# tomvanbraeckel/amv-codec-tools

Hardware: AMD Instinct MI355X
Metric: AMV frames/sec/GPU (160x120 decode, bit-exact) (higher is better)
Workload: dtype int32; 1 GPU; 160x120 AMV decode, 160000-frame synthetic stream per GPU, chunks resident in HBM; parallelism=frame-range x1, frames_per_gpu=160000, stream=seeded synthetic source (BASELINE.md section 4), every frame

## Files before the change

amv-codec-tools_amd/csrc/amv_decode_sync.hip:

```cpp
#include <atomic>

#include "amv_kernels.h"
#include "amv_segment.h"

namespace amv {

namespace {

constexpr uint32_t kRingWords = 16;
constexpr uint32_t kNever = 0xffffffffu;

__device__ __forceinline__ void wave_sync() {
    __builtin_amdgcn_fence(__ATOMIC_SEQ_CST, "wavefront");
    __builtin_amdgcn_wave_barrier();
}

template <int kWidth>
__device__ __forceinline__ uint32_t seg_excl_sum(uint32_t v, uint32_t sub, uint32_t& total) {
    uint32_t x = v;
#pragma unroll
    for (int d = 1; d < kWidth; d <<= 1) {
        const uint32_t y = __shfl_up(x, d, kWidth);
        if (sub >= (uint32_t)d) x += y;
    }
// ... 74 lines not shown
                    }
                }
                wv[q] = make_uint4(w[0], w[1], w[2], w[3]);
            }
#pragma unroll
            for (uint32_t q = 0; q < kBurst; ++q) {
            const uint32_t t0 = b0 + q * kTile;
            if (t0 >= end) break;
            const uint32_t p0 = t0 + lane * 16u;
            const uint32_t w[4] = {wv[q].x, wv[q].y, wv[q].z, wv[q].w};
            uint32_t ff = 0;
#pragma unroll
            for (uint32_t j = 0; j < 4u; ++j) {
                const uint32_t t = ((w[j] & 0x7f7f7f7fu) + 0x01010101u) & w[j] & 0x80808080u;
                ff |= ((((t >> 7) * 0x00204081u) >> 21) & 15u) << (4u * j);
            }
            uint32_t valid = 0xffffu;
            if (t0 == 0u || t0 + kTile > end) {
                const uint32_t lo = first > p0 ? min(first - p0, 16u) : 0u, hi = end > p0 ? min(end - p0, 16u) : 0u;
                valid = ((1u << hi) - 1u) & ~((1u << lo) - 1u);
                ff &= ~((1u << lo) - 1u);
            }
            uint32_t back = wave_shr1(ff);
            if (lane == 0) back = carry;
            const uint32_t before = ((ff << 1) | (back >> 15)) & 0xffffu;
            uint32_t keep;
            if (!__any((ff & before) != 0u || (lane == 0 && (carry >> 14) == 3u))) {
                keep = valid & ~before;
            } else {
                const uint32_t hist = back | (ff << 16);
                keep = 0;
                bool deep = false;
#pragma unroll
                for (uint32_t j = 0; j < 16u; ++j) {
                    const uint32_t run = (uint32_t)__builtin_clz(~(hist << (16u - j)) | 1u);
                    deep = deep || run >= 16u + j;
                    keep |= (!(run & 1u) ? 1u : 0u) << j;
                }
                keep &= valid;
                if (__any(deep)) { retry = true; break; }
            }
            carry = __builtin_amdgcn_readlane(ff, kWave - 1);
            const uint32_t cnt = (uint32_t)__builtin_popcount(keep);
            const uint32_t upto = wave_incl_sum(cnt);
            const uint32_t tile_total = __builtin_amdgcn_readlane(upto, kWave - 1);
            uint32_t d = total + upto - cnt;
#pragma unroll
            for (uint32_t j = 0; j < 4u; ++j) {
                const uint32_t k4 = (keep >> (4u * j)) & 15u;
                const uint32_t packed = __builtin_amdgcn_perm(0u, w[j], s_pack[k4]);
                const uint32_t sh = (d & 3u) * 8u, wd = d >> 2;
                atomicOr(&ring[wd & (kRing - 1u)], packed << sh);
                atomicOr(&ring[(wd + 1u) & (kRing - 1u)], (packed >> 1) >> (31u - sh));
                d += (uint32_t)__builtin_popcount(k4);
            }
            total += tile_total;
            wave_sync();
            const uint32_t whole = total >> 2;
            for (uint32_t x = flushed + lane; x < whole; x += kWave) {
                const uint32_t v = ring[x & (kRing - 1u)];
                ring[x & (kRing - 1u)] = 0u;
                out[x] = __builtin_amdgcn_perm(0u, v, 0x00010203u);
            }
            flushed = whole;
            wave_sync();
            }
        }
        if (!retry) {
            wave_sync();
            const uint32_t x = flushed + lane;
            if (x < ((total + 15u) & ~15u) >> 2) out[x] = __builtin_amdgcn_perm(0u, ring[x & (kRing - 1u)], 0x00010203u);
        }
    }
    if (lane == 0) {
        ws_bytes[frame] = retry ? kNever : total;
        if (retry) retry_list[atomicAdd(retry_count, 1u)] = frame;
    }
}

namespace {

struct Stream {
    const uint32_t* g;
    uint32_t nwords;
    uint32_t* ring;
    uint32_t hi;
    uint4 pf0, pf1;
};

constexpr int kStrideWrite = 8;

__device__ __forceinline__ uint4 stream_piece(const Stream& s, uint32_t x) {
    uint4 v = make_uint4(0, 0, 0, 0);
    if (x < s.nwords) v = *reinterpret_cast<const uint4*>(s.g + x);
    return v;
}

__device__ __forceinline__ void stream_request(Stream& s) {
    s.pf0 = stream_piece(s, s.hi);
    s.pf1 = stream_piece(s, s.hi + 4u);
}

struct SegGeom {
    uint32_t mcu_cols;
    uint32_t per_row;
    uint32_t count;
};

template <uint32_t kFlush>
__device__ __forceinline__ void stage_put(uint32_t* stage, uint32_t pos, uint32_t word) {
    stage[(pos & (2u * kFlush - 1u)) * kWave] = word;
}

template <uint32_t kFlush>
__device__ __forceinline__ void stage_flush(const uint32_t* stage, uint32_t* __restrict__ rec, uint32_t from, uint32_t rec_cap) {
    const uint32_t* p = stage + (from & (2u * kFlush - 1u)) * kWave;
    uint4 v[kFlush / 4u];
#pragma unroll
    for (uint32_t q = 0; q < kFlush / 4u; ++q)
        v[q] = make_uint4(p[(4u * q) * kWave], p[(4u * q + 1u) * kWave], p[(4u * q + 2u) * kWave], p[(4u * q + 3u) * kWave]);
    if (from + kFlush <= rec_cap) {
#pragma unroll
        for (uint32_t q = 0; q < kFlush / 4u; ++q) *reinterpret_cast<uint4*>(rec + from + 4u * q) = v[q];
    }
}

}

struct SyncOut {
    uint32_t* rec;
    const uint32_t* rec_line;
    uint32_t* seg_start;
    uint32_t* lane_tab;
    SegGeom sg;
    uint32_t lane_stride;
    uint32_t* rec_count;
    uint32_t* retry_list;
    uint32_t* retry_count;
    uint32_t ok_in_blocks;
};


namespace {

constexpr uint32_t kFastRegion = kFastWords * 4u;
constexpr uint32_t kFastTableBytes = 4u * kFastRegion;
constexpr uint32_t kServicePace = 4u;
template <int L> constexpr uint32_t skip_pace() { return L >= 16 ? 1u : kServicePace; }
constexpr uint32_t kSlot = kWave * 4u;
constexpr uint32_t kFastRingBytes = (kRingWords + 1u) * kSlot;
constexpr uint32_t kFastSumBytes = 4u * kSlot;
constexpr uint32_t fast_stage_bytes(uint32_t flush) { return 2u * flush * kSlot; }
constexpr uint32_t fast_per_wave(uint32_t flush) { return fast_stage_bytes(flush) + kFastSumBytes + kFastRingBytes; }
constexpr uint32_t fast_waves(uint32_t flush) {
    const uint32_t w = (160u * 1024u - kFastTableBytes) / fast_per_wave(flush);
    return w > 16u ? 16u : w;
}

struct FastState {
    uint32_t t;
    uint32_t k;
    uint32_t j;
    uint32_t togo6;
    uint32_t rp8;
    uint32_t dc;
};

typedef __attribute__((address_space(3))) uint32_t lds_u32;
__device__ __forceinline__ uint32_t lds_get(uint32_t a) { return *(const lds_u32*)(uintptr_t)a; }
__device__ __forceinline__ void lds_put(uint32_t a, uint32_t v) { *(lds_u32*)(uintptr_t)a = v; }
__device__ __forceinline__ uint32_t shl3_add(uint32_t x, uint32_t y) {
    uint32_t d;
    asm("v_lshl_add_u32 %0, %1, 3, %2" : "=v"(d) : "v"(x), "v"(y));
    return d;
}

__device__ __forceinline__ void fast_ring_put(const Stream& s, uint32_t x, const uint4& v) {
    uint32_t* d = s.ring + (x & (kRingWords - 1u)) * kWave;
    d[0] = v.x; d[kWave] = v.y; d[2 * kWave] = v.z; d[3 * kWave] = v.w;
    if ((x & (kRingWords - 1u)) == 0u) s.ring[kRingWords * kWave] = v.x;
}

__device__ __forceinline__ void fast_open(Stream& s) {
    const uint4 a = stream_piece(s, 0u), b = stream_piece(s, 4u), c = stream_piece(s, 8u), d = stream_piece(s, 12u);
    fast_ring_put(s, 0u, a);
    fast_ring_put(s, 4u, b);
    fast_ring_put(s, 8u, c);
    fast_ring_put(s, 12u, d);
    s.hi = kRingWords;
    stream_request(s);
}

template <uint32_t kPace>
__device__ __forceinline__ void fast_service_paced(Stream& s, uint32_t w, bool alive, bool& have, uint32_t stride_no) {
    if (alive && w + 9u > s.hi) {
        do {
            if (!have) stream_request(s);
            fast_ring_put(s, s.hi, s.pf0);
            fast_ring_put(s, s.hi + 4u, s.pf1);
            s.hi += 8u;
            have = false;
        } while (w + 9u > s.hi);
    }
    if ((stride_no & (kPace - 1u)) == 0u) {
        if (alive && !have) {
            stream_request(s);
            have = true;
        }
    }
}

__device__ __forceinline__ uint32_t fast_window(uint32_t ringb, uint32_t t) {
    const uint32_t ra = shl3_add(t & 0x1e0u, ringb);
    return __builtin_amdgcn_alignbit(lds_get(ra), lds_get(ra + kSlot), ~t);
}

__device__ __forceinline__ uint32_t fast_lookup(const FastState& s, uint32_t v) {
    const uint32_t toff = (((3u * kFastRegion) >> s.j) & kFastRegion) | (~s.dc & (2u * kFastRegion));
    const uint32_t e1 = lds_get(((v >> 21) & 0x7fcu) | toff);
    const uint32_t x2 = max(v >> 16, kFastLongFirst - 1u);
    const uint32_t e2 = lds_get((x2 << 2) + (toff + (kFastM2Word * 4u - 4u * (kFastLongFirst - 1u))));
    return e1 | e2;
}

template <uint32_t kFlush, bool kLimit>
__device__ __forceinline__ void fast_stride(uint32_t ringb, uint32_t stageb, uint32_t sumb, uint32_t lim1, FastState& s, uint32_t& seen,
                                            uint32_t& worst) {
#pragma unroll
    for (int it = 0; it < kStrideWrite; ++it) {
        const uint32_t ca = (((2u * kSlot) >> s.j) & (3u * kSlot)) | sumb;
        const uint32_t sum = lds_get(ca);
        const uint32_t v = fast_window(ringb, s.t);
        __builtin_amdgcn_sched_barrier(0);
        uint32_t run = (uint32_t)((int32_t)s.togo6 >> 31);
        if (kLimit) run &= (uint32_t)((int32_t)(s.t - lim1) >> 31);
        const uint32_t e = fast_lookup(s, v) & run;
        seen |= e;
        const uint32_t used = e >> 24;
        const int x = __builtin_amdgcn_sbfe((int)v, 0u - used, e);
        const uint32_t full = __builtin_amdgcn_ubfe(0xffffffffu, 0u, e);
        const uint32_t val = (uint32_t)x - (full ^ (uint32_t)(x >> 31));
        s.t += used;
        const uint32_t kn = s.k + ((e >> 16) & 255u);
        worst = min(worst, kn - 65u);
        uint32_t dcn = (uint32_t)__builtin_amdgcn_sbfe((int)kn, 6u, 1u);
        asm("" : "+v"(dcn));
        lds_put(ca, sum + (val & s.dc));
        const uint32_t rv = val + (sum & s.dc);
        lds_put((s.rp8 & ((2u * kFlush - 1u) << 8)) | stageb, (rv << 16) | (s.togo6 & 0xfc0u) | (kn - 1u));
        s.rp8 += e & kFastEmit;
        s.k = kn & ~dcn;
        s.togo6 += kn & 64u;
        s.j = min(s.j + dcn, 5u);
        s.dc = dcn;
    }
}

template <bool kLimit>
__device__ __forceinline__ uint32_t fast_replay(uint32_t ringb, uint32_t lim1, FastState& s) {
    for (int it = 0; it < kStrideWrite; ++it) {
        if (s.togo6 == 0u) break;
        if (kLimit && (int32_t)(s.t - lim1) >= 0) break;
        const uint32_t e = fast_lookup(s, fast_window(ringb, s.t));
        if (e & kFastInvalid) return 1u;
        const uint32_t kn = s.k + ((e >> 16) & 255u);
        s.t += e >> 24;
        if (kn - 65u < 15u) return 2u;
        const bool end = (kn & 64u) != 0u;
        s.rp8 += e & kFastEmit;
        s.k = end ? 0u : kn;
        s.togo6 += kn & 64u;
        s.j = end ? (s.j == 0u ? 5u : s.j - 1u) : s.j;
        s.dc = end ? ~0u : 0u;
    }
    return 0u;
}

__device__ __forceinline__ void fast_open_at(Stream& s, uint32_t w) {
    const uint32_t lo = w & ~7u;
    const uint4 a = stream_piece(s, lo), b = stream_piece(s, lo + 4u), c = stream_piece(s, lo + 8u), d = stream_piece(s, lo + 12u);
    fast_ring_put(s, lo, a);
    fast_ring_put(s, lo + 4u, b);
    fast_ring_put(s, lo + 8u, c);
    fast_ring_put(s, lo + 12u, d);
    s.hi = lo + kRingWords;
    stream_request(s);
}

template <uint32_t kPace>
__device__ __forceinline__ void fast_skip(Stream& win, uint32_t ringb, FastState& s, uint32_t lim1, uint32_t& nblk6, uint32_t& nrec8) {
    nblk6 = nrec8 = 0u;
    bool active = (int32_t)(s.t - lim1) < 0;
    if (!__ballot(active)) return;
    fast_open_at(win, active ? (s.t + 1u) >> 5 : 0u);
    bool have = true;
    uint32_t stride_no = 1u;
    while (__ballot(active) != 0ull) {
        fast_service_paced<kPace>(win, (s.t + 1u) >> 5, active, have, stride_no++);
#pragma unroll
        for (int it = 0; it < kStrideWrite; ++it) {
            const uint32_t v = fast_window(ringb, s.t);
            const uint32_t e = fast_lookup(s, v) & (uint32_t)((int32_t)(s.t - lim1) >> 31);
            s.t += e >> 24;
            const uint32_t kn = s.k + ((e >> 16) & 255u);
            uint32_t dcn = (uint32_t)__builtin_amdgcn_sbfe((int)kn, 6u, 1u);
            asm("" : "+v"(dcn));
            nrec8 += e & kFastEmit;
            nblk6 += kn & 64u;
            s.k = kn & ~dcn;
            s.j = min(s.j + dcn, 5u);
            s.dc = dcn;
        }
        active = (int32_t)(s.t - lim1) < 0;
    }
}

}

template <uint32_t kFlush>
__global__ __launch_bounds__(kWave * 16) void amv_huffman_fast_kernel(
    const uint32_t* __restrict__ ws, const uint32_t* __restrict__ ws_bytes, uint32_t n,
    const uint32_t* __restrict__ list, const uint32_t* __restrict__ list_count,
    uint32_t blocks_per_frame, const uint32_t* __restrict__ ws_line,
    const HuffDecodeImage* __restrict__ img, SyncOut out, int32_t* __restrict__ status,
    uint32_t* __restrict__ nmcu_ok, uint32_t* __restrict__ queue, unsigned long long* __restrict__ stats) {
    static_assert(kFlush == 8u, "amv_huffman_fast_kernel stages a stride's eight record slots");
    extern __shared__ __attribute__((aligned(16))) uint8_t s_mem[];
    const uint32_t wave = threadIdx.x >> 6, lane = threadIdx.x & 63u, nwaves = blockDim.x >> 6;
    {
        const uint4* src = reinterpret_cast<const uint4*>(&img->fast[0][0]);
        uint4* dst = reinterpret_cast<uint4*>(s_mem);
        for (uint32_t i = threadIdx.x; i < kFastTableBytes / 16u; i += blockDim.x) dst[i] = src[i];
    }
    __syncthreads();
    const bool lds_at_zero = (uint32_t)(uintptr_t)(__attribute__((address_space(3))) uint8_t*)s_mem == 0u;
    const uint32_t stageb = kFastTableBytes + wave * fast_stage_bytes(kFlush) + lane * 4u;
    const uint32_t sumb = kFastTableBytes + nwaves * fast_stage_bytes(kFlush) + wave * kFastSumBytes + lane * 4u;
    const uint32_t ringb = kFastTableBytes + nwaves * (fast_stage_bytes(kFlush) + kFastSumBytes) + wave * kFastRingBytes + lane * 4u;
    uint32_t* const stage = reinterpret_cast<uint32_t*>(s_mem + stageb);
    if (list) n = *list_count;
    const uint32_t ntasks = (n + kWave - 1) / kWave;
    const SegGeom sg = out.sg;
    for (;;) {
        uint32_t task = 0;
        if (lane == 0) task = atomicAdd(queue, 1u);
        task = __shfl(task, 0);
        if (task >= ntasks) return;
        const uint32_t idx = task * kWave + lane;
        const uint32_t frame = idx < n ? (list ? list[idx] : idx) : kNever;
        uint32_t total = frame != kNever ? ws_bytes[frame] : kNever;
        if (!lds_at_zero && total != kNever) {
            out.retry_list[atomicAdd(out.retry_count, 1u)] = frame;
            total = kNever;
        }
        if (frame != kNever && total == kNever) out.rec_count[frame] = kNever;
        if (!lds_at_zero) continue;
        const bool live = total != kNever;
        const uint32_t fsafe = live ? frame : 0u;
        const uint32_t line0 = out.rec_line[fsafe];
        uint32_t* const rec = out.rec + (uint64_t)line0 * 32u;
        const uint32_t line1 = out.rec_line[fsafe + 1u];
        const uint32_t cap_rec = line1 > line0 ? (line1 - line0) * 32u : 0u;
        uint2* const seg_out = reinterpret_cast<uint2*>(out.seg_start) + (uint64_t)fsafe * (sg.count + 1u);
        const uint32_t valid_bits = live ? total * 8u : 0u;
        Stream win{ws + (uint64_t)ws_line[fsafe] * 4u, live ? ((total + 15u) >> 4) * 4u : 0u, reinterpret_cast<uint32_t*>(s_mem + ringb), 0u,
                   make_uint4(0, 0, 0, 0), make_uint4(0, 0, 0, 0)};
        fast_open(win);
        for (uint32_t c = 0; c < 3u; ++c) lds_put(sumb + c * kSlot, 0u);

        FastState s{0xffffffffu, 0u, 5u, live ? 0u - (blocks_per_frame << 6) : 0u, 0u, ~0u};
        bool alive = live;
        uint32_t stop = 0;
        uint32_t stride_no = 0;
        bool have_words = true;
        uint32_t recpos = 0;
        uint32_t seg_next = 0, seg_col = 0, seg_blk = 0;
        uint32_t end_blocks = 0;
#pragma unroll
        for (uint32_t q = 0; q < 2u * kFlush; ++q) stage_put<kFlush>(stage, q, kDummyRecord);
        if (__ballot(alive) != 0ull) do {
            const bool line_live = alive;
            uint4 line[8];
#pragma unroll
            for (int quarter = 0; quarter < 4; ++quarter) {
                fast_service_paced<kServicePace>(win, (s.t + 1u) >> 5, alive, have_words, stride_no);
                const bool running = alive;
                s.rp8 = stride_no << 11;
                const FastState start = s;
                uint32_t worst = ~0u, seen = 0u;
                fast_stride<kFlush, false>(ringb, stageb, sumb, 0u, s, seen, worst);
                const bool trouble = alive && (worst < 15u || (seen & kFastInvalid) != 0u);
                if (__ballot(trouble) != 0ull) {
                    if (trouble) {
                        s = start;
                        stop = fast_replay<false>(ringb, 0u, s);
                        alive = false;
                        for (uint32_t q = s.rp8 >> 8; q < stride_no * 8u + 8u; ++q) stage_put<kFlush>(stage, q, kDummyRecord);
                    }
                }
                if (alive && s.togo6 == 0u) { stop = 3u; alive = false; }
                stage_put<kFlush>(stage, s.rp8 >> 8, kDummyRecord);
                {
                    uint32_t* p = stage + ((stride_no & 1u) * kFlush) * kWave;
                    line[2 * quarter] = make_uint4(p[0], p[kWave], p[2 * kWave], p[3 * kWave]);
                    line[2 * quarter + 1] = make_uint4(p[4 * kWave], p[5 * kWave], p[6 * kWave], p[7 * kWave]);
#pragma unroll
                    for (uint32_t q = 0; q < 8u; ++q) p[q * kWave] = kDummyRecord;
                }
                bool hit = false;
                uint32_t blocks = 0;
                if (running) {
                    blocks = blocks_per_frame + (uint32_t)((int32_t)s.togo6 >> 6);
                    hit = seg_next < sg.count && blocks + (s.k ? 1u : 0u) > seg_blk;
                    if (!alive) { end_blocks = blocks; s.togo6 = 0u; }
                }
                if (__ballot(hit) != 0ull) {
                    if (hit) {
                        seg_out[seg_next++] = make_uint2(start.rp8 >> 8, s.rp8 >> 8);
                        const bool last = seg_col + 1u == sg.per_row;
                        seg_blk += 6u * (last ? sg.mcu_cols - seg_col * kSegMcus : kSegMcus);
                        seg_col = last ? 0u : seg_col + 1u;
                    }
                }
                ++stride_no;
            }
            if (line_live) {
                const uint32_t at = (stride_no - 4u) * 8u;
                if (at + 32u <= cap_rec) {
                    uint4* d = reinterpret_cast<uint4*>(rec + at);
#pragma unroll
                    for (int q = 0; q < 8; ++q) d[q] = line[q];
                }
                recpos = at + 32u;
            }
        } while (__ballot(alive) != 0ull);
        if (live) {
            const uint32_t bits = s.t + 1u + (stop == 1u ? 17u : 0u);
            uint32_t st = stop == 1u ? kStFormat : (stop == 2u ? kStOverrun : 0u);
            if (bits > valid_bits) st |= kStTruncated;
            reinterpret_cast<uint4*>(out.lane_tab)[(uint64_t)frame * out.lane_stride] = make_uint4(0u, 0u, 0u, 0u);
            for (uint32_t m = seg_next; m <= sg.count; ++m) seg_out[m] = make_uint2(recpos, recpos);
            if (stats) atomicAdd(&stats[0], 1ull);
            if (recpos > cap_rec) {
                out.rec_count[frame] = kNever;
                out.retry_list[atomicAdd(out.retry_count, 1u)] = frame;
            } else {
                status[frame] = (int32_t)st;
                nmcu_ok[frame] = out.ok_in_blocks ? end_blocks : end_blocks / 6u;
                out.rec_count[frame] = recpos;
            }
        }
    }
}

template <int L>
__global__ __launch_bounds__(kWave * 16) void amv_huffman_sync2_kernel(
    const uint32_t* __restrict__ ws, const uint32_t* __restrict__ ws_bytes, uint32_t n,
    const uint32_t* __restrict__ list, const uint32_t* __restrict__ list_count,
    uint32_t blocks_per_frame, const uint32_t* __restrict__ ws_line,
    const HuffDecodeImage* __restrict__ img, SyncOut out, int32_t* __restrict__ status,
    uint32_t* __restrict__ nmcu_ok, uint32_t* __restrict__ queue, unsigned long long* __restrict__ stats) {
    constexpr int kFrames = kWave / L;
    constexpr uint32_t kFlush = 8u;
    constexpr uint32_t kNoLimit = 0x7ffffffeu;
    extern __shared__ __attribute__((aligned(16))) uint8_t s_mem[];
    const uint32_t wave = threadIdx.x >> 6, lane = threadIdx.x & 63u, nwaves = blockDim.x >> 6;
    const uint32_t slot = lane / L, sub = lane % L;
    if (list && *list_count == 0u) return;
    {
        const uint4* src = reinterpret_cast<const uint4*>(&img->fast[0][0]);
        uint4* dst = reinterpret_cast<uint4*>(s_mem);
        for (uint32_t i = threadIdx.x; i < kFastTableBytes / 16u; i += blockDim.x) dst[i] = src[i];
    }
    __syncthreads();
    const bool lds_at_zero = (uint32_t)(uintptr_t)(__attribute__((address_space(3))) uint8_t*)s_mem == 0u;
    const uint32_t stageb = kFastTableBytes + wave * fast_stage_bytes(kFlush) + lane * 4u;
    const uint32_t sumb = kFastTableBytes + nwaves * fast_stage_bytes(kFlush) + wave * kFastSumBytes + lane * 4u;
    const uint32_t ringb = kFastTableBytes + nwaves * (fast_stage_bytes(kFlush) + kFastSumBytes) + wave * kFastRingBytes + lane * 4u;
    uint32_t* const stage = reinterpret_cast<uint32_t*>(s_mem + stageb);
    if (list) n = *list_count;
    const uint32_t ntasks = (n + kFrames - 1) / kFrames;
    const SegGeom sg = out.sg;
    for (;;) {
        uint32_t task = 0;
        if (lane == 0) task = atomicAdd(queue, 1u);
        task = __shfl(task, 0);
        if (task >= ntasks) return;

        const bool timing = stats != nullptr && lane == 0;
        unsigned long long tc[6] = {0, 0, 0, 0, 0, 0};
        unsigned long long wall0 = 0;
        if (timing) { tc[0] = tc[1] = clock64(); wall0 = wall_clock64(); }

        const uint32_t idx = task * kFrames + slot;
        const uint32_t frame = idx < n ? (list ? list[idx] : idx) : kNever;
        uint32_t total = frame != kNever ? ws_bytes[frame] : kNever;
        if (!lds_at_zero && total != kNever) {
            if (sub == 0) out.retry_list[atomicAdd(out.retry_count, 1u)] = frame;
            total = kNever;
        }
        if (frame != kNever && total == kNever && sub == 0) out.rec_count[frame] = kNever;
        if (!lds_at_zero) continue;
        const bool live = total != kNever;
        const uint32_t fsafe = live ? frame : 0u;
        const uint32_t line0 = out.rec_line[fsafe];
        uint32_t* const rec = out.rec + (uint64_t)line0 * 32u;
        const uint32_t line1 = out.rec_line[fsafe + 1u];
        const uint32_t cap_rec = line1 > line0 ? (line1 - line0) * 32u : 0u;
        uint2* const seg_out = reinterpret_cast<uint2*>(out.seg_start) + (uint64_t)fsafe * (sg.count + 1u);
        const uint32_t valid_bits = live ? total * 8u : 0u;
        Stream win{ws + (uint64_t)ws_line[fsafe] * 4u, live ? ((total + 15u) >> 4) * 4u : 0u, reinterpret_cast<uint32_t*>(s_mem + ringb), 0u,
                   make_uint4(0, 0, 0, 0), make_uint4(0, 0, 0, 0)};

        uint32_t S = ((valid_bits + L - 1) / L + 31u) & ~31u;
        if (S < 64u) S = 64u;
        constexpr uint32_t kMemo = 5u, kPend = 4u;
        constexpr uint32_t kGuess = 5u << 11;
        const uint32_t stage0 = stageb - lane * 4u, sum0 = sumb - lane * 4u, col0 = slot * L;
        const uint64_t seg = L == 64 ? ~0ull : (((1ull << (L & 63)) - 1ull) << (slot * L));
        auto col_addr = [&](uint32_t col, uint32_t w) { return (w < 16u ? stage0 + w * kSlot : sum0 + (w - 16u) * kSlot) + col * 4u; };
        const bool walks = live && sub != L - 1;
        uint32_t my_blocks6 = 0u, my_recs8 = 0u, seeded = 0u, rounds = 0u;
        lds_put(col_addr(lane, 19u), 0u);
        {
            FastState st{sub * S - 1u, 0u, 5u, 0u, 0u, ~0u};
            const uint32_t lim1 = walks ? (sub + 1u) * S - 1u : 0u;
            if (!walks) st.t = lim1;
            uint32_t b6, r8;
            fast_skip<skip_pace<L>()>(win, ringb, st, lim1, b6, r8);
            if (walks) {
                lds_put(col_addr(lane, 0u), kGuess | (((st.t - lim1) | (st.k << 5) | (st.j << 11)) << 16));
                lds_put(col_addr(lane, 1u), b6);
                lds_put(col_addr(lane, 2u), r8);
                lds_put(col_addr(lane, 19u), 1u);
            }
        }
        if (timing) tc[2] = clock64();
        constexpr uint32_t kNone = 7u;
        uint32_t final_at = kNone, final_code = kGuess;
        bool settled = !live;
        for (int round = 0; round < L + 1; ++round) {
            wave_sync();
            const uint32_t held = lds_get(col_addr(lane, 19u));
            const uint32_t left_n = sub ? lds_get(col_addr(lane - 1u, 19u)) : 0u;
            uint32_t mine[kMemo], cand[kMemo];
#pragma unroll
            for (uint32_t q = 0; q < kMemo; ++q) {
                const uint32_t a = lds_get(col_addr(lane, 3u * q)), b = lds_get(col_addr(sub ? lane - 1u : lane, 3u * q));
                mine[q] = q < held ? a : kNever;
                cand[q] = q < left_n ? b >> 16 : kNever;
            }
            uint32_t link = (kNone << 15) | (kNone << 18) | (kNone << 21);
#pragma unroll
            for (uint32_t qp = 0; qp < kMemo; ++qp) {
                uint32_t to = kNone;
#pragma unroll
                for (uint32_t q = 0; q < kMemo; ++q) to = (mine[q] != kNever && (mine[q] & 0xffffu) == cand[qp]) ? q : to;
                if (sub == L - 1) to = cand[qp] != kNever ? 0u : kNone;
                link |= to << (3u * qp);
            }
            if (sub == 0) link = 0u;
            if (!live) link = 0u;
#pragma unroll
            for (int d = 1; d < L; d <<= 1) {
                const uint32_t before = __shfl_up(link, d, L);
                uint32_t both = 0u;
#pragma unroll
                for (uint32_t f = 0; f < 8u; ++f) both |= ((link >> (3u * ((before >> (3u * f)) & 7u))) & 7u) << (3u * f);
                if (sub >= (uint32_t)d) link = both;
            }
            final_at = link & 7u;
// ... 96 lines not shown
        uint32_t all_blocks, all_recs;
        const uint32_t blk0 = seg_excl_sum<L>(my_blocks6 >> 6, sub, all_blocks);
        const uint32_t rec0 = seg_excl_sum<L>(((my_recs8 >> 8) + kFlush - 1u) & ~(kFlush - 1u), sub, all_recs);

        for (uint32_t c = 0; c < 3u; ++c) lds_put(sumb + c * kSlot, 0u);
        FastState s = entry;
        s.togo6 = (blk0 - blocks_per_frame) << 6;
        s.rp8 = rec0 << 8;
        bool alive = live && blk0 < blocks_per_frame;
        if (!alive) s.togo6 = 0u;
        const uint32_t wlim1 = sub == L - 1 ? kNoLimit : (sub + 1u) * S - 1u;
        const uint32_t dc_first = blk0 + (s.k ? 1u : 0u);
        uint32_t stop = 0;
        uint32_t flushed = rec0;
        uint32_t end_blocks = 0;
        uint32_t seg_next, seg_col, seg_blk;
        {
            const uint32_t m_first = (dc_first + 5u) / 6u;
            uint32_t row = m_first / sg.mcu_cols;
            const uint32_t col = m_first - row * sg.mcu_cols;
            seg_col = (col + kSegMcus - 1u) / kSegMcus;
            if (seg_col >= sg.per_row) { ++row; seg_col = 0u; }
            seg_next = row * sg.per_row + seg_col;
            seg_blk = (row * sg.mcu_cols + seg_col * kSegMcus) * 6u;
        }
        if (__ballot(alive) != 0ull) {
        fast_open_at(win, alive ? (s.t + 1u) >> 5 : 0u);
        bool have_words = true;
        uint32_t stride_no = 1u;
        do {
            fast_service_paced<kServicePace>(win, (s.t + 1u) >> 5, alive, have_words, stride_no++);
            if ((s.rp8 >> 8) - flushed >= kFlush) {
                stage_flush<kFlush>(stage, rec, flushed, cap_rec);
                flushed += kFlush;
            }
            const bool running = alive;
            const FastState start = s;
            uint32_t worst = ~0u, seen = 0u;
            fast_stride<kFlush, true>(ringb, stageb, sumb, wlim1, s, seen, worst);
            const bool trouble = alive && (worst < 15u || (seen & kFastInvalid) != 0u);
            if (__ballot(trouble) != 0ull) {
                if (trouble) {
                    s = start;
                    stop = fast_replay<true>(ringb, wlim1, s);
                    alive = false;
                }
            }
            if (alive && s.togo6 == 0u) { stop = 3u; alive = false; }
            if (alive && (int32_t)(s.t - wlim1) >= 0) alive = false;
            bool hit = false;
            if (running) {
                const uint32_t blocks = blocks_per_frame + (uint32_t)((int32_t)s.togo6 >> 6);
                hit = seg_next < sg.count && blocks + (s.k ? 1u : 0u) > seg_blk;
                if (!alive) { end_blocks = blocks; s.togo6 = 0u; }
            }
            if (__ballot(hit) != 0ull) {
                if (hit) {
                    seg_out[seg_next++] = make_uint2(start.rp8 >> 8, s.rp8 >> 8);
                    const bool last = seg_col + 1u == sg.per_row;
                    seg_blk += 6u * (last ? sg.mcu_cols - seg_col * kSegMcus : kSegMcus);
                    seg_col = last ? 0u : seg_col + 1u;
                }
            }
        } while (__ballot(alive) != 0ull);
        }
        const uint32_t recpos = s.rp8 >> 8;
        {
            const uint32_t end = (recpos + kFlush - 1u) & ~(kFlush - 1u);
            for (uint32_t q = recpos; q < end; ++q) stage_put<kFlush>(stage, q, kDummyRecord);
            while (flushed < end) {
                stage_flush<kFlush>(stage, rec, flushed, cap_rec);
                flushed += kFlush;
            }
        }
        if (timing) tc[4] = clock64();
        const uint32_t err = stop == 1u ? kStFormat : (stop == 2u ? kStOverrun : 0u);
        const uint32_t stop_p = s.t + 1u + (stop == 1u ? 17u : 0u);
        const uint64_t stop_mask = __ballot(stop != 0u) & seg;
        uint32_t st = 0, good_blocks = blocks_per_frame, rec_total = 0, seg_seen = 0;
        int stop_lane = 0;
        if (stop_mask) {
            stop_lane = __builtin_ctzll(stop_mask);
            const uint32_t e = __shfl(err, stop_lane);
            const uint32_t eb = __shfl(end_blocks, stop_lane);
            const uint32_t sp = __shfl(stop_p, stop_lane);
            rec_total = __shfl(recpos, stop_lane);
            seg_seen = __shfl(seg_next, stop_lane);
            st = e;
            if (e) good_blocks = eb;
            if (sp > valid_bits) st |= kStTruncated;
        } else {
            st = kStFormat; good_blocks = 0;
        }

        uint32_t tot;
        const uint32_t by = seg_excl_sum<L>(lds_get(sumb), sub, tot);
        const uint32_t bu = seg_excl_sum<L>(lds_get(sumb + kSlot), sub, tot);
        const uint32_t bv = seg_excl_sum<L>(lds_get(sumb + 2u * kSlot), sub, tot);
        if (live) {
            const bool real = (int)lane <= stop_lane && blk0 < blocks_per_frame;
            reinterpret_cast<uint4*>(out.lane_tab)[(uint64_t)frame * out.lane_stride + sub] = make_uint4(real ? dc_first : kNever, by, bu, bv);
            for (uint32_t m = seg_seen + sub; m <= sg.count; m += L) seg_out[m] = make_uint2(rec_total, rec_total);
        }
        uint32_t wave_rounds = rounds;
        if (stats) {
#pragma unroll
            for (int off = 32; off; off >>= 1) wave_rounds = max(wave_rounds, (uint32_t)__shfl_xor((int)wave_rounds, off));
        }
        if (timing) {
            tc[5] = clock64();
            for (int q = 0; q < 5; ++q) atomicAdd(&stats[4 + q], tc[q + 1] - tc[q]);
            atomicAdd(&stats[9], 1ull);
            if (task < kTraceTasks) {
                unsigned long long* tr = stats + kTraceBase + (unsigned long long)task * 8ull;
                tr[0] = wall0;
                tr[1] = wall_clock64();
                for (int q = 0; q < 4; ++q) tr[2 + q] = tc[q + 2] - tc[q + 1];
                tr[6] = wave_rounds | (unsigned long long)S << 32;
                tr[7] = (unsigned long long)blockIdx.x << 32 | (unsigned long long)wave << 16 | (unsigned long long)L;
            }
        }
        if (live && sub == 0) {
            if (stats) {
                atomicAdd(&stats[0], 1ull);
                atomicAdd(&stats[1], (unsigned long long)rounds);
                atomicMax(&stats[2], (unsigned long long)rounds);
            }
            if (rec_total > cap_rec || unsettled) {
                out.rec_count[frame] = kNever;
                out.retry_list[atomicAdd(out.retry_count, 1u)] = frame;
            } else {
                status[frame] = (int32_t)st;
                nmcu_ok[frame] = out.ok_in_blocks ? good_blocks : good_blocks / 6u;
                out.rec_count[frame] = rec_total | ((uint32_t)(L - 1) << 24);
            }
        }
    }
}

namespace {

template <uint32_t kFlush>
void launch_fast(const uint32_t* ws, const uint32_t* ws_bytes, uint32_t n, const uint32_t* list,
                 const uint32_t* list_count, const FrameGeom& g, const uint32_t* ws_line,
                 const HuffDecodeImage* d_img, const SyncOut& out, int32_t* status, uint32_t* nmcu_ok,
                 uint32_t* queue, unsigned long long* stats, uint32_t cus, hipStream_t s) {
    constexpr uint32_t kMaxWaves = fast_waves(kFlush);
    static std::atomic<uint64_t> raised{0};
    int dev = 0;
    (void)hipGetDevice(&dev);
    const uint64_t bit = 1ull << (dev & 63);
    if (!(raised.load(std::memory_order_relaxed) & bit)) {
        (void)hipFuncSetAttribute(reinterpret_cast<const void*>(amv_huffman_fast_kernel<kFlush>),
                                  hipFuncAttributeMaxDynamicSharedMemorySize, (int)(kFastTableBytes + kMaxWaves * fast_per_wave(kFlush)));
        raised.fetch_or(bit, std::memory_order_relaxed);
    }
    const uint32_t tasks = (n + (uint32_t)kWave - 1u) / (uint32_t)kWave;
    uint32_t waves = (tasks + cus - 1u) / cus;
    if (waves < 4u) waves = 4u;
    if (waves > kMaxWaves) waves = kMaxWaves;
    const uint32_t grid = tasks < cus ? tasks : cus;
    hipLaunchKernelGGL((amv_huffman_fast_kernel<kFlush>), dim3(grid), dim3(kWave * waves), kFastTableBytes + waves * fast_per_wave(kFlush), s,
                       ws, ws_bytes, n, list, list_count, g.blocks, ws_line, d_img, out, status, nmcu_ok, queue, stats);
}

template <int L>
void launch_sync2(const uint32_t* ws, const uint32_t* ws_bytes, uint32_t n, const uint32_t* list,
                  const uint32_t* list_count, const FrameGeom& g, const uint32_t* ws_line,
                  const HuffDecodeImage* d_img, const SyncOut& out, int32_t* status, uint32_t* nmcu_ok,
                  uint32_t* queue, unsigned long long* stats, uint32_t cus, hipStream_t s) {
    constexpr uint32_t kMaxWaves = fast_waves(8u);
    static std::atomic<uint64_t> raised{0};
    int dev = 0;
    (void)hipGetDevice(&dev);
    const uint64_t bit = 1ull << (dev & 63);
    if (!(raised.load(std::memory_order_relaxed) & bit)) {
        (void)hipFuncSetAttribute(reinterpret_cast<const void*>(amv_huffman_sync2_kernel<L>),
                                  hipFuncAttributeMaxDynamicSharedMemorySize, (int)(kFastTableBytes + kMaxWaves * fast_per_wave(8u)));
        raised.fetch_or(bit, std::memory_order_relaxed);
    }
    const uint32_t tasks = (n + (uint32_t)(kWave / L) - 1u) / (uint32_t)(kWave / L);
    uint32_t waves = (tasks + cus - 1u) / cus;
    if (waves < 4u) waves = 4u;
    if (waves > kMaxWaves) waves = kMaxWaves;
    const uint32_t grid = tasks < cus ? tasks : cus;
    hipLaunchKernelGGL((amv_huffman_sync2_kernel<L>), dim3(grid), dim3(kWave * waves), kFastTableBytes + waves * fast_per_wave(8u), s, ws,
                       ws_bytes, n, list, list_count, g.blocks, ws_line, d_img, out, status, nmcu_ok, queue, stats);
}

}

int huffman_sync_lanes(uint32_t n, uint32_t cus, int wanted, uint64_t pixels) {
    if (wanted == 1 || wanted == 2 || wanted == 4 || wanted == 8 || wanted == 16 || wanted == 32 || wanted == 64) return wanted;
    if (n >= cus * 230u) return 1;
    if (n >= cus * 150u) return 2;
    const uint64_t resident = (uint64_t)cus * fast_waves(8u);
    if (pixels <= 30000u && (uint64_t)n * 8u > resident * 64u) return 2;
    int full = 8;
    while (full < 64 && (uint64_t)full * 25000u <= pixels) full *= 2;
    int fill = 8;
    if (n <= resident) fill = 64;
    else if (n <= 2u * resident) fill = 32;
    else if (n <= 4u * resident) fill = 16;
    int cap = 8;
    while (cap < 64 && (uint64_t)cap * 2u * 500u <= pixels) cap *= 2;
    if (n <= cus * 5u) cap = 64;
    if (fill > cap) fill = cap;
    return fill > full ? fill : full;
}

__global__ __launch_bounds__(256) void amv_split_kernel(const uint32_t* __restrict__ lens, uint32_t n, const uint32_t* __restrict__ ws_line,
                                                        uint32_t* __restrict__ heavy, uint32_t* __restrict__ light, uint32_t* __restrict__ count) {
    const uint32_t i = blockIdx.x * 256u + threadIdx.x, lane = threadIdx.x & 63u;
    const bool in = i < n;
    const uint64_t all = ws_line[n];
    const bool is_heavy = in && (((uint64_t)lens[in ? i : 0u] + 47u) >> 4) * n > 2u * all;
    const uint64_t hm = __ballot(is_heavy), lm = __ballot(in && !is_heavy);
    uint32_t hb = 0u, lb = 0u;
    if (lane == 0u) {
        if (hm) hb = atomicAdd(&count[0], (uint32_t)__builtin_popcountll(hm));
        if (lm) lb = atomicAdd(&count[1], (uint32_t)__builtin_popcountll(lm));
    }
    hb = (uint32_t)__shfl((int)hb, 0);
    lb = (uint32_t)__shfl((int)lb, 0);
    const uint64_t below = (1ull << lane) - 1ull;
    if (is_heavy) heavy[hb + (uint32_t)__builtin_popcountll(hm & below)] = i;
    else if (in) light[lb + (uint32_t)__builtin_popcountll(lm & below)] = i;
}

void launch_split_by_weight(const uint32_t* lens, uint32_t n, const uint32_t* ws_line, uint32_t* heavy, uint32_t* light, uint32_t* count,
                            hipStream_t s) {
    if (n == 0) return;
    hipLaunchKernelGGL(amv_split_kernel, dim3((n + 255u) / 256u), dim3(256), 0, s, lens, n, ws_line, heavy, light, count);
}

void launch_unstuff(const uint8_t* blob, uint64_t blob_bytes, const uint64_t* offs, const uint32_t* lens, uint32_t n,
                    const uint32_t* ws_line, uint32_t* ws, uint32_t* ws_bytes, uint32_t* retry_list, uint32_t* retry_count,
                    hipStream_t s) {
    if (n == 0) return;
    hipLaunchKernelGGL(amv_unstuff_kernel, dim3((n + 3u) / 4u), dim3(256), 0, s, blob, blob_bytes, offs, lens, n,
                       ws_line, ws, ws_bytes, retry_list, retry_count);
}

void launch_huffman_sync(const uint32_t* ws, const uint32_t* ws_bytes, uint32_t n, const uint32_t* list,
                         const uint32_t* list_count, const FrameGeom& g, const uint32_t* ws_line, int lanes_per_frame,
                         const HuffDecodeImage* d_img, const SyncSinks& sinks, int32_t* status, uint32_t* nmcu_ok,
                         uint32_t* queue, unsigned long long* stats, uint32_t cus, hipStream_t s) {
    if (n == 0) return;
    const uint32_t per_row = segs_per_row(g);
    SyncOut out{sinks.rec, sinks.rec_line, sinks.seg_start, sinks.lane_tab, SegGeom{g.mcu_cols, per_row, per_row * g.mcu_rows},
                sinks.lanes, sinks.rec_count, sinks.retry_list, sinks.retry_count, sinks.ok_in_blocks};
#define AMV_SYNC_ARGS ws, ws_bytes, n, list, list_count, g, ws_line, d_img, out, status, nmcu_ok, queue, stats, cus, s
    switch (lanes_per_frame) {
        case 64: launch_sync2<64>(AMV_SYNC_ARGS); break;
        case 32: launch_sync2<32>(AMV_SYNC_ARGS); break;
        case 8: launch_sync2<8>(AMV_SYNC_ARGS); break;
        case 4: launch_sync2<4>(AMV_SYNC_ARGS); break;
        case 2: launch_sync2<2>(AMV_SYNC_ARGS); break;
        case 1: launch_fast<8>(AMV_SYNC_ARGS); break;
        default: launch_sync2<16>(AMV_SYNC_ARGS); break;
    }
#undef AMV_SYNC_ARGS
}

namespace {
constexpr uint32_t kLayoutBlock = 256;

__device__ __forceinline__ uint32_t layout_lines(uint32_t len, const LayoutSpec& sp) {
    const uint64_t want = ((uint64_t)len * sp.per_byte_x2 >> 1) + sp.add;
    return (uint32_t)((min(want, (uint64_t)sp.hi) + ((1u << sp.unit_shift) - 1u)) >> sp.unit_shift);
}

struct Sum2 { uint64_t x, y; };
__device__ __forceinline__ Sum2 block_scan2(uint2 v, Sum2* s_wave, Sum2& tot) {
    const uint32_t lane = threadIdx.x & 63u, wave = threadIdx.x >> 6;
    Sum2 inc{v.x, v.y};
#pragma unroll
    for (int d = 1; d < 64; d <<= 1) {
        const uint64_t ax = (uint64_t)__shfl_up((unsigned long long)inc.x, d), ay = (uint64_t)__shfl_up((unsigned long long)inc.y, d);
        if (lane >= (uint32_t)d) { inc.x += ax; inc.y += ay; }
    }
    if (lane == 63u) s_wave[wave] = inc;
    __syncthreads();
    Sum2 base{0u, 0u};
    tot = Sum2{0u, 0u};
    for (uint32_t k = 0; k < kLayoutBlock / 64u; ++k) {
        const Sum2 w = s_wave[k];
        if (k < wave) { base.x += w.x; base.y += w.y; }
        tot.x += w.x; tot.y += w.y;
    }
    return Sum2{base.x + inc.x - v.x, base.y + inc.y - v.y};
}
__device__ __forceinline__ uint32_t sat32(uint64_t v) { return (uint32_t)min(v, (uint64_t)0xffffffffu); }
}

__global__ __launch_bounds__(kLayoutBlock) void amv_layout_sums_kernel(const uint32_t* __restrict__ lens, uint32_t n, LayoutSpec a, LayoutSpec b,
                                                                      uint2* __restrict__ sums) {
    __shared__ Sum2 s_wave[kLayoutBlock / 64u];
    const uint32_t i = blockIdx.x * kLayoutBlock + threadIdx.x;
    const uint32_t len = i < n ? lens[i] : 0u;
    Sum2 tot;
    (void)block_scan2(i < n ? make_uint2(layout_lines(len, a), b.line ? layout_lines(len, b) : 0u) : make_uint2(0u, 0u), s_wave, tot);
    if (threadIdx.x == 0u) sums[blockIdx.x] = make_uint2(sat32(tot.x), sat32(tot.y));
}

__global__ __launch_bounds__(1024) void amv_layout_scan_kernel(uint2* __restrict__ sums, uint32_t nb, uint32_t cap_a, uint32_t cap_b) {
    __shared__ uint64_t s_x[1024], s_y[1024];
    const uint32_t per = (nb + 1023u) / 1024u;
    const uint32_t lo = min(threadIdx.x * per, nb), up = min(lo + per, nb);
    uint64_t mx = 0, my = 0;
    for (uint32_t i = lo; i < up; ++i) { mx += sums[i].x; my += sums[i].y; }
    s_x[threadIdx.x] = mx; s_y[threadIdx.x] = my;
    __syncthreads();
    for (uint32_t d = 1; d < 1024u; d <<= 1) {
        const uint64_t lx = threadIdx.x >= d ? s_x[threadIdx.x - d] : 0u, ly = threadIdx.x >= d ? s_y[threadIdx.x - d] : 0u;
// ... 120 lines not shown
```

amv-codec-tools_amd/csrc/amv_tables.h:

```cpp
#pragma once
#include <stdint.h>

namespace amv {

static constexpr uint8_t kQuantLuma[64] = {
    8,  6,  6,  7,  6,  5,  8,  7,  7,  7,  9,  9,  8,  10, 12, 20, 13, 12, 11, 11, 12, 25,
    18, 19, 15, 20, 29, 26, 31, 30, 29, 26, 28, 28, 32, 36, 46, 39, 32, 34, 44, 39, 28, 28,
    40, 55, 41, 44, 48, 49, 52, 52, 52, 31, 39, 57, 61, 56, 50, 60, 46, 51, 52, 50};
static constexpr uint8_t kQuantChroma[64] = {
    9,  9,  9,  12, 11, 12, 24, 13, 13, 24, 50, 33, 28, 33, 50, 50, 50, 50, 50, 50, 50, 50,
    50, 50, 50, 50, 50, 50, 50, 50, 50, 50, 50, 50, 50, 50, 50, 50, 50, 50, 50, 50, 50, 50,
    50, 50, 50, 50, 50, 50, 50, 50, 50, 50, 50, 50, 50, 50, 50, 50, 50, 50, 50, 50};

static constexpr uint8_t kQ60Luma[64] = {
    13, 9,  10, 11, 10, 8,  13, 11, 10, 11, 14, 14, 13, 15, 19, 32, 21, 19, 18, 18, 19, 39,
    28, 30, 23, 32, 46, 41, 49, 48, 46, 41, 45, 44, 51, 58, 74, 62, 51, 54, 70, 55, 44, 45,
    64, 87, 65, 70, 76, 78, 82, 83, 82, 50, 62, 90, 97, 90, 80, 96, 74, 81, 82, 79};
static constexpr uint8_t kQ60Chroma[64] = {
    14, 14, 14, 19, 17, 19, 38, 21, 21, 38, 79, 53, 45, 53, 79, 79, 79, 79, 79, 79, 79, 79,
    79, 79, 79, 79, 79, 79, 79, 79, 79, 79, 79, 79, 79, 79, 79, 79, 79, 79, 79, 79, 79, 79,
    79, 79, 79, 79, 79, 79, 79, 79, 79, 79, 79, 79, 79, 79, 79, 79, 79, 79, 79, 79};

static constexpr uint8_t kScanOfNatural[64] = {
    0,  1,  5,  6,  14, 15, 27, 28, 2,  4,  7,  13, 16, 26, 29, 42, 3,  8,  12, 17, 25, 30,
    41, 43, 9,  11, 18, 24, 31, 40, 44, 53, 10, 19, 23, 32, 39, 45, 52, 54, 20, 22, 33, 38,
    46, 51, 55, 60, 21, 34, 37, 47, 50, 56, 59, 61, 35, 36, 48, 49, 57, 58, 62, 63};
static constexpr int kAmvlibQuirkNatural = 3 * 8 + 4;
static constexpr int kAmvlibQuirkScan = 37;

static constexpr uint8_t kHuffCount[4][16] = {
    {0, 1, 5, 1, 1, 1, 1, 1, 1, 0, 0, 0, 0, 0, 0, 0},
    {0, 3, 1, 1, 1, 1, 1, 1, 1, 1, 1, 0, 0, 0, 0, 0},
    {0, 2, 1, 3, 3, 2, 4, 3, 5, 5, 4, 4, 0, 0, 1, 0x7d},
    {0, 2, 1, 2, 4, 4, 3, 4, 7, 5, 4, 4, 0, 1, 2, 0x77}};
static constexpr uint8_t kHuffDcSymbols[12] = {0, 1, 2, 3, 4, 5, 6, 7, 8, 9, 10, 11};
static constexpr uint8_t kHuffAcLumaSymbols[162] = {
    0x01, 0x02, 0x03, 0x00, 0x04, 0x11, 0x05, 0x12, 0x21, 0x31, 0x41, 0x06, 0x13, 0x51, 0x61,
    0x07, 0x22, 0x71, 0x14, 0x32, 0x81, 0x91, 0xa1, 0x08, 0x23, 0x42, 0xb1, 0xc1, 0x15, 0x52,
    0xd1, 0xf0, 0x24, 0x33, 0x62, 0x72, 0x82, 0x09, 0x0a, 0x16, 0x17, 0x18, 0x19, 0x1a, 0x25,
    0x26, 0x27, 0x28, 0x29, 0x2a, 0x34, 0x35, 0x36, 0x37, 0x38, 0x39, 0x3a, 0x43, 0x44, 0x45,
    0x46, 0x47, 0x48, 0x49, 0x4a, 0x53, 0x54, 0x55, 0x56, 0x57, 0x58, 0x59, 0x5a, 0x63, 0x64,
    0x65, 0x66, 0x67, 0x68, 0x69, 0x6a, 0x73, 0x74, 0x75, 0x76, 0x77, 0x78, 0x79, 0x7a, 0x83,
    0x84, 0x85, 0x86, 0x87, 0x88, 0x89, 0x8a, 0x92, 0x93, 0x94, 0x95, 0x96, 0x97, 0x98, 0x99,
    0x9a, 0xa2, 0xa3, 0xa4, 0xa5, 0xa6, 0xa7, 0xa8, 0xa9, 0xaa, 0xb2, 0xb3, 0xb4, 0xb5, 0xb6,
    0xb7, 0xb8, 0xb9, 0xba, 0xc2, 0xc3, 0xc4, 0xc5, 0xc6, 0xc7, 0xc8, 0xc9, 0xca, 0xd2, 0xd3,
    0xd4, 0xd5, 0xd6, 0xd7, 0xd8, 0xd9, 0xda, 0xe1, 0xe2, 0xe3, 0xe4, 0xe5, 0xe6, 0xe7, 0xe8,
    0xe9, 0xea, 0xf1, 0xf2, 0xf3, 0xf4, 0xf5, 0xf6, 0xf7, 0xf8, 0xf9, 0xfa};
static constexpr uint8_t kHuffAcChromaSymbols[162] = {
    0x00, 0x01, 0x02, 0x03, 0x11, 0x04, 0x05, 0x21, 0x31, 0x06, 0x12, 0x41, 0x51, 0x07, 0x61,
    0x71, 0x13, 0x22, 0x32, 0x81, 0x08, 0x14, 0x42, 0x91, 0xa1, 0xb1, 0xc1, 0x09, 0x23, 0x33,
    0x52, 0xf0, 0x15, 0x62, 0x72, 0xd1, 0x0a, 0x16, 0x24, 0x34, 0xe1, 0x25, 0xf1, 0x17, 0x18,
    0x19, 0x1a, 0x26, 0x27, 0x28, 0x29, 0x2a, 0x35, 0x36, 0x37, 0x38, 0x39, 0x3a, 0x43, 0x44,
    0x45, 0x46, 0x47, 0x48, 0x49, 0x4a, 0x53, 0x54, 0x55, 0x56, 0x57, 0x58, 0x59, 0x5a, 0x63,
    0x64, 0x65, 0x66, 0x67, 0x68, 0x69, 0x6a, 0x73, 0x74, 0x75, 0x76, 0x77, 0x78, 0x79, 0x7a,
    0x82, 0x83, 0x84, 0x85, 0x86, 0x87, 0x88, 0x89, 0x8a, 0x92, 0x93, 0x94, 0x95, 0x96, 0x97,
    0x98, 0x99, 0x9a, 0xa2, 0xa3, 0xa4, 0xa5, 0xa6, 0xa7, 0xa8, 0xa9, 0xaa, 0xb2, 0xb3, 0xb4,
    0xb5, 0xb6, 0xb7, 0xb8, 0xb9, 0xba, 0xc2, 0xc3, 0xc4, 0xc5, 0xc6, 0xc7, 0xc8, 0xc9, 0xca,
    0xd2, 0xd3, 0xd4, 0xd5, 0xd6, 0xd7, 0xd8, 0xd9, 0xda, 0xe2, 0xe3, 0xe4, 0xe5, 0xe6, 0xe7,
    0xe8, 0xe9, 0xea, 0xf2, 0xf3, 0xf4, 0xf5, 0xf6, 0xf7, 0xf8, 0xf9, 0xfa};

static constexpr int8_t kImaIndexAdjust[16] = {-1, -1, -1, -1, 2, 4, 6, 8, -1, -1, -1, -1, 2, 4, 6, 8};
static constexpr int16_t kImaStep[89] = {
    7,     8,     9,     10,    11,    12,    13,    14,    16,    17,    19,    21,    23,
    25,    28,    31,    34,    37,    41,    45,    50,    55,    60,    66,    73,    80,
    88,    97,    107,   118,   130,   143,   157,   173,   190,   209,   230,   253,   279,
    307,   337,   371,   408,   449,   494,   544,   598,   658,   724,   796,   876,   963,
    1060,  1166,  1282,  1411,  1552,  1707,  1878,  2066,  2272,  2499,  2749,  3024,  3327,
    3660,  4026,  4428,  4871,  5358,  5894,  6484,  7132,  7845,  8630,  9493,  10442, 11487,
    12635, 13899, 15289, 16818, 18500, 20350, 22385, 24623, 27086, 29794, 32767};

static constexpr int16_t kSinQ14[65] = {
    0,     402,   804,   1205,  1606,  2006,  2404,  2801,  3196,  3590,  3981,  4370,  4756,
    5139,  5520,  5897,  6270,  6639,  7005,  7366,  7723,  8076,  8423,  8765,  9102,  9434,
    9760,  10080, 10394, 10702, 11003, 11297, 11585, 11866, 12140, 12406, 12665, 12916, 13160,
    13395, 13623, 13842, 14053, 14256, 14449, 14635, 14811, 14978, 15137, 15286, 15426, 15557,
    15679, 15791, 15893, 15986, 16069, 16143, 16207, 16261, 16305, 16340, 16364, 16379, 16384};


static constexpr int kLut1Bits = 9;
static constexpr int kLut2Bits = 7;
static constexpr int kLut2Pages = 16;
static constexpr uint32_t kFastWords = 2048;
static constexpr uint32_t kFastM2Word = 512;
static constexpr uint32_t kFastLongFirst = 0xfc00u;
static constexpr uint32_t kFastInvalid = 1u << 5, kFastEmit = 1u << 8, kFastEobAdvance = 192u;
struct HuffDecodeImage {
    uint16_t l1[4][1 << kLut1Bits];
    uint16_t l2[kLut2Pages][1 << kLut2Bits];
    uint32_t fast[4][kFastWords];
};

struct HuffEncodeImage {
    uint32_t code[4][256];
};

struct FrameGeom {
    uint32_t width, height;
    uint32_t stride;
    uint32_t mcu_cols;
    uint32_t mcu_rows;
    uint32_t mcus;
    uint32_t blocks;
    uint64_t frame_bytes;
};

inline FrameGeom make_geom(uint32_t w, uint32_t h) {
    FrameGeom g;
    g.width = w;
    g.height = h;
    g.stride = (w * 24 + 31) / 32 * 4;
    g.mcu_cols = (w + 15) / 16;
    g.mcu_rows = (h + 15) / 16;
    g.mcus = g.mcu_cols * g.mcu_rows;
    g.blocks = g.mcus * 6;
    g.frame_bytes = (uint64_t)g.stride * h;
    return g;
}

}
```

Measured before the change: 30.44 million frames/s.

## Keep stride records in registers instead of LDS staging buffer

The Huffman fast kernel now writes each stride's eight record words into per-lane registers instead of scattering them into a per-wave LDS staging area and reading them back. Table entries are rewritten while loading into LDS so that invalid codes and no-value symbols are encoded in the entry itself, which lets a single min-based check detect trouble. The aim is to cut LDS traffic, LDS footprint and the per-stride dummy refills. The cost is higher register pressure, and dummy padding now covers every slot in the stride rather than only the emitted ones.

```diff
diff --git a/amv-codec-tools_amd/csrc/amv_decode_sync.hip b/amv-codec-tools_amd/csrc/amv_decode_sync.hip
--- a/amv-codec-tools_amd/csrc/amv_decode_sync.hip
+++ b/amv-codec-tools_amd/csrc/amv_decode_sync.hip
@@ -250,6 +250,7 @@
 constexpr uint32_t kFastSumBytes = 4u * kSlot;
 constexpr uint32_t fast_stage_bytes(uint32_t flush) { return 2u * flush * kSlot; }
 constexpr uint32_t fast_per_wave(uint32_t flush) { return fast_stage_bytes(flush) + kFastSumBytes + kFastRingBytes; }
+constexpr uint32_t lane_per_wave() { return kFastSumBytes + kFastRingBytes; }
 constexpr uint32_t fast_waves(uint32_t flush) {
     const uint32_t w = (160u * 1024u - kFastTableBytes) / fast_per_wave(flush);
     return w > 16u ? 16u : w;
@@ -313,7 +314,8 @@
     return __builtin_amdgcn_alignbit(lds_get(ra), lds_get(ra + kSlot), ~t);
 }
 
-__device__ __forceinline__ uint32_t fast_lookup(const FastState& s, uint32_t v) {
+template <class State>
+__device__ __forceinline__ uint32_t fast_lookup(const State& s, uint32_t v) {
     const uint32_t toff = (((3u * kFastRegion) >> s.j) & kFastRegion) | (~s.dc & (2u * kFastRegion));
     const uint32_t e1 = lds_get(((v >> 21) & 0x7fcu) | toff);
     const uint32_t x2 = max(v >> 16, kFastLongFirst - 1u);
@@ -374,6 +376,57 @@
     return 0u;
 }
 
+struct LaneState {
+    uint32_t t, k, j, togo6, dc;
+};
+
+__device__ __forceinline__ void lane_stride(uint32_t ringb, uint32_t sumb, LaneState& s, uint32_t& worst, uint32_t (&w)[kStrideWrite]) {
+#pragma unroll
+    for (int it = 0; it < kStrideWrite; ++it) {
+        const uint32_t ca = (((2u * kSlot) >> s.j) & (3u * kSlot)) | sumb;
+        const uint32_t sum = lds_get(ca);
+        const uint32_t v = fast_window(ringb, s.t);
+        __builtin_amdgcn_sched_barrier(0);
+        const uint32_t run = (uint32_t)((int32_t)s.togo6 >> 31);
+        const uint32_t e = fast_lookup(s, v) & run;
+        uint32_t fill = e | ~run;
+        asm("" : "+v"(fill));
+        const uint32_t used = e >> 24;
+        const int x = __builtin_amdgcn_sbfe((int)v, 0u - used, e);
+        const uint32_t full = __builtin_amdgcn_ubfe(0xffffffffu, 0u, e);
+        const uint32_t val = (uint32_t)x - (full ^ (uint32_t)(x >> 31));
+        s.t += used;
+        const uint32_t kn = s.k + ((e >> 16) & 255u);
+        worst = min(worst, kn - 65u);
+        uint32_t dcn = (uint32_t)__builtin_amdgcn_sbfe((int)kn, 6u, 1u);
+        asm("" : "+v"(dcn));
+        lds_put(ca, sum + (val & s.dc));
+        const uint32_t rv = val + (sum & s.dc);
+        w[it] = (rv << 16) | ((fill & kFastNoValue) | ((s.togo6 & 0xfc0u) | __builtin_elementwise_sub_sat(kn, 1u)));
+        s.k = kn & ~dcn;
+        s.togo6 += kn & 64u;
+        s.j = min(s.j + dcn, 5u);
+        s.dc = dcn;
+    }
+}
+
+__device__ __forceinline__ uint32_t lane_replay(uint32_t ringb, LaneState& s, uint32_t& taken) {
+    for (taken = 0u; taken < (uint32_t)kStrideWrite; ++taken) {
+        if (s.togo6 == 0u) break;
+        const uint32_t e = fast_lookup(s, fast_window(ringb, s.t));
+        if (e & kFastInvalid) return 1u;
+        const uint32_t kn = s.k + ((e >> 16) & 255u);
+        s.t += e >> 24;
+        if (kn - 65u < 15u) return 2u;
+        const bool end = (kn & 64u) != 0u;
+        s.k = end ? 0u : kn;
+        s.togo6 += kn & 64u;
+        s.j = end ? (s.j == 0u ? 5u : s.j - 1u) : s.j;
+        s.dc = end ? ~0u : 0u;
+    }
+    return 0u;
+}
+
 __device__ __forceinline__ void fast_open_at(Stream& s, uint32_t w) {
     const uint32_t lo = w & ~7u;
     const uint4 a = stream_piece(s, lo), b = stream_piece(s, lo + 4u), c = stream_piece(s, lo + 8u), d = stream_piece(s, lo + 12u);
@@ -422,20 +475,21 @@
     uint32_t blocks_per_frame, const uint32_t* __restrict__ ws_line,
     const HuffDecodeImage* __restrict__ img, SyncOut out, int32_t* __restrict__ status,
     uint32_t* __restrict__ nmcu_ok, uint32_t* __restrict__ queue, unsigned long long* __restrict__ stats) {
-    static_assert(kFlush == 8u, "amv_huffman_fast_kernel stages a stride's eight record slots");
+    static_assert(kFlush == 8u && kStrideWrite == 8, "amv_huffman_fast_kernel puts a stride's eight words into a quarter of a line");
     extern __shared__ __attribute__((aligned(16))) uint8_t s_mem[];
     const uint32_t wave = threadIdx.x >> 6, lane = threadIdx.x & 63u, nwaves = blockDim.x >> 6;
     {
         const uint4* src = reinterpret_cast<const uint4*>(&img->fast[0][0]);
         uint4* dst = reinterpret_cast<uint4*>(s_mem);
-        for (uint32_t i = threadIdx.x; i < kFastTableBytes / 16u; i += blockDim.x) dst[i] = src[i];
+        for (uint32_t i = threadIdx.x; i < kFastTableBytes / 16u; i += blockDim.x) {
+            const uint4 e = src[i];
+            dst[i] = make_uint4(fast_strict_entry(e.x), fast_strict_entry(e.y), fast_strict_entry(e.z), fast_strict_entry(e.w));
+        }
     }
     __syncthreads();
     const bool lds_at_zero = (uint32_t)(uintptr_t)(__attribute__((address_space(3))) uint8_t*)s_mem == 0u;
-    const uint32_t stageb = kFastTableBytes + wave * fast_stage_bytes(kFlush) + lane * 4u;
-    const uint32_t sumb = kFastTableBytes + nwaves * fast_stage_bytes(kFlush) + wave * kFastSumBytes + lane * 4u;
-    const uint32_t ringb = kFastTableBytes + nwaves * (fast_stage_bytes(kFlush) + kFastSumBytes) + wave * kFastRingBytes + lane * 4u;
-    uint32_t* const stage = reinterpret_cast<uint32_t*>(s_mem + stageb);
+    const uint32_t sumb = kFastTableBytes + wave * kFastSumBytes + lane * 4u;
+    const uint32_t ringb = kFastTableBytes + nwaves * kFastSumBytes + wave * kFastRingBytes + lane * 4u;
     if (list) n = *list_count;
     const uint32_t ntasks = (n + kWave - 1) / kWave;
     const SegGeom sg = out.sg;
@@ -466,7 +520,7 @@
         fast_open(win);
         for (uint32_t c = 0; c < 3u; ++c) lds_put(sumb + c * kSlot, 0u);
 
-        FastState s{0xffffffffu, 0u, 5u, live ? 0u - (blocks_per_frame << 6) : 0u, 0u, ~0u};
+        LaneState s{0xffffffffu, 0u, 5u, live ? 0u - (blocks_per_frame << 6) : 0u, ~0u};
         bool alive = live;
         uint32_t stop = 0;
         uint32_t stride_no = 0;
@@ -474,8 +528,6 @@
         uint32_t recpos = 0;
         uint32_t seg_next = 0, seg_col = 0, seg_blk = 0;
         uint32_t end_blocks = 0;
-#pragma unroll
-        for (uint32_t q = 0; q < 2u * kFlush; ++q) stage_put<kFlush>(stage, q, kDummyRecord);
         if (__ballot(alive) != 0ull) do {
             const bool line_live = alive;
             uint4 line[8];
@@ -483,28 +535,25 @@
             for (int quarter = 0; quarter < 4; ++quarter) {
                 fast_service_paced<kServicePace>(win, (s.t + 1u) >> 5, alive, have_words, stride_no);
                 const bool running = alive;
-                s.rp8 = stride_no << 11;
-                const FastState start = s;
-                uint32_t worst = ~0u, seen = 0u;
-                fast_stride<kFlush, false>(ringb, stageb, sumb, 0u, s, seen, worst);
-                const bool trouble = alive && (worst < 15u || (seen & kFastInvalid) != 0u);
+                const LaneState start = s;
+                uint32_t worst = ~0u;
+                uint32_t w[kStrideWrite];
+                lane_stride(ringb, sumb, s, worst, w);
+                const bool trouble = alive && worst < kFastStrictBad;
                 if (__ballot(trouble) != 0ull) {
                     if (trouble) {
                         s = start;
-                        stop = fast_replay<false>(ringb, 0u, s);
+                        uint32_t taken;
+                        stop = lane_replay(ringb, s, taken);
                         alive = false;
-                        for (uint32_t q = s.rp8 >> 8; q < stride_no * 8u + 8u; ++q) stage_put<kFlush>(stage, q, kDummyRecord);
+#pragma unroll
+                        for (uint32_t q = 0; q < (uint32_t)kStrideWrite; ++q)
+                            if (q >= taken) w[q] = kDummyRecord;
                     }
                 }
                 if (alive && s.togo6 == 0u) { stop = 3u; alive = false; }
-                stage_put<kFlush>(stage, s.rp8 >> 8, kDummyRecord);
-                {
-                    uint32_t* p = stage + ((stride_no & 1u) * kFlush) * kWave;
-                    line[2 * quarter] = make_uint4(p[0], p[kWave], p[2 * kWave], p[3 * kWave]);
-                    line[2 * quarter + 1] = make_uint4(p[4 * kWave], p[5 * kWave], p[6 * kWave], p[7 * kWave]);
-#pragma unroll
-                    for (uint32_t q = 0; q < 8u; ++q) p[q * kWave] = kDummyRecord;
-                }
+                line[2 * quarter] = make_uint4(w[0], w[1], w[2], w[3]);
+                line[2 * quarter + 1] = make_uint4(w[4], w[5], w[6], w[7]);
                 bool hit = false;
                 uint32_t blocks = 0;
                 if (running) {
@@ -514,7 +563,7 @@
                 }
                 if (__ballot(hit) != 0ull) {
                     if (hit) {
-                        seg_out[seg_next++] = make_uint2(start.rp8 >> 8, s.rp8 >> 8);
+                        seg_out[seg_next++] = make_uint2(stride_no * 8u, stride_no * 8u + 8u);
                         const bool last = seg_col + 1u == sg.per_row;
                         seg_blk += 6u * (last ? sg.mcu_cols - seg_col * kSegMcus : kSegMcus);
                         seg_col = last ? 0u : seg_col + 1u;
@@ -917,7 +966,7 @@
     const uint64_t bit = 1ull << (dev & 63);
     if (!(raised.load(std::memory_order_relaxed) & bit)) {
         (void)hipFuncSetAttribute(reinterpret_cast<const void*>(amv_huffman_fast_kernel<kFlush>),
-                                  hipFuncAttributeMaxDynamicSharedMemorySize, (int)(kFastTableBytes + kMaxWaves * fast_per_wave(kFlush)));
+                                  hipFuncAttributeMaxDynamicSharedMemorySize, (int)(kFastTableBytes + kMaxWaves * lane_per_wave()));
         raised.fetch_or(bit, std::memory_order_relaxed);
     }
     const uint32_t tasks = (n + (uint32_t)kWave - 1u) / (uint32_t)kWave;
@@ -925,7 +974,7 @@
     if (waves < 4u) waves = 4u;
     if (waves > kMaxWaves) waves = kMaxWaves;
     const uint32_t grid = tasks < cus ? tasks : cus;
-    hipLaunchKernelGGL((amv_huffman_fast_kernel<kFlush>), dim3(grid), dim3(kWave * waves), kFastTableBytes + waves * fast_per_wave(kFlush), s,
+    hipLaunchKernelGGL((amv_huffman_fast_kernel<kFlush>), dim3(grid), dim3(kWave * waves), kFastTableBytes + waves * lane_per_wave(), s,
                        ws, ws_bytes, n, list, list_count, g.blocks, ws_line, d_img, out, status, nmcu_ok, queue, stats);
 }
 
diff --git a/amv-codec-tools_amd/csrc/amv_tables.h b/amv-codec-tools_amd/csrc/amv_tables.h
--- a/amv-codec-tools_amd/csrc/amv_tables.h
+++ b/amv-codec-tools_amd/csrc/amv_tables.h
@@ -84,6 +84,12 @@
 static constexpr uint32_t kFastM2Word = 512;
 static constexpr uint32_t kFastLongFirst = 0xfc00u;
 static constexpr uint32_t kFastInvalid = 1u << 5, kFastEmit = 1u << 8, kFastEobAdvance = 192u;
+static constexpr uint32_t kFastNoValue = 1u << 15, kFastInvalidAdvance = 128u, kFastStrictBad = 127u;
+constexpr uint32_t fast_strict_entry(uint32_t e) {
+    if (e == 0u) return 0u;
+    if (e & kFastInvalid) e = (e & ~(255u << 16)) | (kFastInvalidAdvance << 16);
+    return (e & kFastEmit) ? e : (e | kFastNoValue);
+}
 struct HuffDecodeImage {
     uint16_t l1[4][1 << kLut1Bits];
     uint16_t l2[kLut2Pages][1 << kLut2Bits];
```

Measured after the change: 30.54 million frames/s (median of 6 runs). Within noise of the previous version (+0.3%).
